# ChanukyaVardhan/Video-Moment-Localization

Hardware: AMD Instinct MI355X
Metric: proposals/sec (fwd+bwd) (higher is better)
Workload: dtype f32; 1 GPU; activitynet_t256: SMIN T=256 L=64 C=4 d=512 dl=128 Nq=20 Din=500 layers=3, batch 64/GPU, default init seed 43; step = zero_grad+fwd+restated loss+bwd+Adam (torch fused); global_batch=64, parallelism=dp1, dist_world_size=1

## Files before the change

include/smin_hip.h:

```cpp
#ifndef SMIN_HIP_H
#define SMIN_HIP_H
#include <stddef.h>
#include <stdint.h>

#ifdef __cplusplus
extern "C" {
#endif

#define SMIN_HIP_ABI_VERSION 2

int smin_abi_version(void);
int smin_set_gemm_mode(int mode);
int smin_get_gemm_mode(void);
#define SMIN_PROF_MOMENT_FWD 1
#define SMIN_PROF_MOMENT_DX 2
#define SMIN_PROF_MOMENT_DW 3
#define SMIN_PROF_ATTN_FWD 4
#define SMIN_PROF_ATTN_BWD 5
int smin_prof_enable(int on);
int smin_prof_read(int32_t* tags, float* ms, int cap);
const char* smin_target_arch(void);
size_t smin_workspace_bytes(int N, int B, int C, int D, int dl, int Nq);

int smin_proposal_map_fwd(void* stream, const float* f, const int32_t* cells, int N, int B, int T, int L, int C, int D,
// ... 155 lines not shown
                              int N, int B, int L, int C, int dl, int Nq,
                              const float* Mq, const float* uq, const float* what, const float* shat, const float* qmask,
                              uint16_t* cc_h, float* ccmean);
int smin_content_attn_fwd_probs(void* stream, const float* chat, const int32_t* cells, const int32_t* row_ptr,
                                int N, int B, int L, int C, int dl, int Nq,
                                const float* Mq, const float* uq, const float* what, const float* shat, const float* qmask,
                                void* cc, int cc_bf16, float* ccmean, float* probs);
int smin_content_attn_maps_dense(void* stream, const float* probs, const int32_t* cellmap, const int32_t* cells,
                                 int B, int L, int C, int dl, int Nq, const float* uq, const float* qmask, float* out);
#define SMIN_ATTN_MAPS_MAX_LAYERS 8
int smin_attn_maps_gather(void* stream, const float* const* probs, const float* const* bmaps, int nl, const int32_t* cellmap,
                          const int64_t* idx, int B, int L, int C, int Nq, int k, float* content, float* boundary);
size_t smin_content_attn_bwd_workspace_bytes(int N, int B, int C, int dl);
int smin_content_attn_bwd(void* stream, const float* dcc, const float* dccmean, const float* chat,
                          const int32_t* cells, const int32_t* row_ptr, int N, int B, int L, int C, int dl, int Nq,
                          const float* Mq, const float* uq, const float* what, const float* shat, const float* qmask,
                          float* dchat, float* dMq, float* duq, float* dwhat, float* dshat, void* ws, size_t ws_bytes);

int smin_linear_rows_fwd(void* stream, const float* const* xs, int nseg, const float* W, const float* bias, const float* add_rows,
                         const float* add_cells, int C, int R, int O, int K, float* y);
size_t smin_linear_rows_bwd_workspace_bytes(int R, int O, int Ktot);
int smin_linear_rows_bwd(void* stream, const float* dy, const float* const* xs, int nseg, const float* WT, int R, int O, int K,
                         float* const* dxs, float* dW, float* dbias, void* ws, size_t ws_bytes);
int smin_linear_rows_fwd_xh(void* stream, const uint16_t* const* xs, int nseg, const float* W, const float* bias, const float* add_rows,
                            const float* add_cells, int C, int R, int O, int K, float* y);
int smin_linear_rows_bwd_xh(void* stream, const float* dy, const uint16_t* const* xs, int nseg, int R, int O, int K,
                            float* dW, float* dbias, void* ws, size_t ws_bytes);
int smin_linear_rows_dx_acc(void* stream, const float* dy, int nseg, const float* WT, int R, int O, int K, float* const* dxs);
int smin_group_sum(void* stream, const float* x, int groups, int C, int W, float* out);

int smin_word_prep_fwd(void* stream, const float* fw, const float* fs, const float* qmask, const float* const* params, int nl, int B, int Nq, int D,
                       int dl, float* what, float* shat, float* kb, float* Mq, float* uq);
size_t smin_word_prep_bwd_workspace_bytes(int nl, int B, int Nq, int D, int dl);
int smin_word_prep_bwd(void* stream, const float* const* dwhat, const float* const* dshat, const float* const* dMq, const float* const* duq,
                       const float* fw, const float* fs, const float* qmask, const float* what, const float* kb, const float* const* params,
                       int nl, int B, int Nq, int D, int dl, float* dfw, float* dfs, float* const* dparams, void* ws, size_t ws_bytes);

int smin_video_encoder_fwd(void* stream, const float* x, const float* W, const float* bias, const float* pe, const float* vmask,
                           const float* fs, int B, int T, int Din, int D, float* fv, float* f);
int smin_video_encoder_gate(void* stream, const float* fv, const float* fs, int B, int T, int D, float* f);
size_t smin_video_encoder_bwd_workspace_bytes(int B, int T, int Din, int D);
int smin_video_encoder_bwd(void* stream, const float* df, const float* fv, const float* fs, const float* vmask, const float* x,
                           int B, int T, int Din, int D, float* dW, float* dbias, float* dpe, float* dfs, void* ws, size_t ws_bytes);
int smin_video_encoder_bwd_input(void* stream, const float* WT, const float* vmask, int B, int T, int Din, int D, float* dx,
                                 const void* ws, size_t ws_bytes);

int smin_sentence_feature_fwd(void* stream, const float* fw, const int32_t* len, int B, int Nq, int H, float* fs);
int smin_sentence_feature_bwd(void* stream, const float* dfs, const int32_t* len, int B, int Nq, int H, float* dfw);
int smin_lstm_pack(void* stream, const float* const* w, int In, int H, float* Wih, float* bias, float* Whh, float* W4);
int smin_lstm_pack_layers(void* stream, int nlayers, const float* const* w, const int* In, int H, float* const* Wih, float* const* bias,
                          float* const* Whh, float* const* W4);
int smin_bilstm_layer_fwd(void* stream, const float* X, const float* Wih_cat, const float* bias_cat, const float* W4,
                          const int32_t* len, int B, int Nq, int In, int H, float* G, float* Hout, float* Cs);
size_t smin_bilstm_layer_bwd_workspace_bytes(int B, int Nq, int In, int H);
int smin_bilstm_layer_bwd(void* stream, const float* dHout, const float* X, const float* Hout, const float* G, const float* Cs,
                          const float* Wih_catT, const float* Whh, const int32_t* len, int B, int Nq, int In, int H,
                          float* dX, float* dWih_cat, float* dbias_cat, float* dWhh, void* ws, size_t ws_bytes);
int smin_bilstm_layer_bwd_weights(void* stream, int which, const float* X, const float* Hout, int B, int Nq, int In, int H,
                                  float* dWih_cat, float* dbias_cat, float* dbias_cat2, float* dWhh, void* ws, size_t ws_bytes);

int smin_lstm_cluster_error(void);

int smin_build_cells(void* stream, const uint8_t* mask, int B, int L, int all_cells,
                     int32_t* cells, int32_t* row_ptr, int32_t* cellmap);
int smin_build_cells_n(void* stream, const uint8_t* mask, int B, int L, int all_cells, int n_expected,
                       int32_t* cells, int32_t* row_ptr, int32_t* cellmap, int32_t* status);
// ... 78 lines not shown
```

video-moment-localization_amd/csrc/torch_binding.cpp:

```cpp
#include <ATen/ATen.h>
#include <c10/hip/HIPGuard.h>
#include <c10/hip/HIPStream.h>
#include <hip/hip_runtime_api.h>
#include <torch/csrc/autograd/custom_function.h>
#include <torch/library.h>
#include <ATen/core/dispatch/Dispatcher.h>
#include <ATen/core/stack.h>

#include <cmath>
#include <map>
#include <mutex>
#include <tuple>
#include <vector>

#include "smin_hip.h"

namespace {

using at::Tensor;
using torch::autograd::AutogradContext;
using torch::autograd::variable_list;
using HStream = c10::hip::HIPStream;

#define SMIN_CK(call)                                                                           \
// ... 957 lines not shown
                    auto ws = scratch(smin_linear_rows_bwd_workspace_bytes(n, dl, D), dev);
                    SMIN_CK(smin_linear_rows_bwd(cur(), fp(dhp), xs, 1, nullptr, n, dl, D, nullptr, fpm(dWch), nullptr, ws.p, ws.n));
                    if (prep_kernel) base_ch[k] = dWch; else acc(dprm.layer(k, L_CH_W), dWch);
                }
            }
            {
                std::vector<Tensor> later;
                for (int64_t kk = k + 1; kk < nl; ++kk) later.push_back(dHs[kk]);
                std::vector<const float*> dh{fp(dcum)}, dr{fp(dfm)};
                Tensor later_sum;
                if (later.size() <= 3) for (auto& t : later) dh.push_back(fp(t));
                else { later_sum = sum_list(later); dh.push_back(fp(later_sum)); }
                if (k == 0) dr.push_back(fp(dcum));
                Tensor dfm_k = at::empty({N, D}, opt), dfs = at::empty_like(fs);
                auto ws = scratch((size_t)4 * B * 512 * D + 4096, dev);
                SMIN_CK(smin_gate_bwd(cur(), dh.data(), i32(dh.size()), dr.data(), i32(dr.size()), fp(ls.fm), fp(fs), ip(row_ptr), n, B, Li, D, fpm(dfm_k), fpm(dfs), ws.p, ws.n,
                                      ip(cells), fp(ls.A), fp(dbu)));
                dfs_parts.push_back(dfs);
                dfm = dfm_k;
            }
            dcum_next = dcum; dfb_next = dfb_k;
        }

        hipStreamCaptureStatus capture = hipStreamCaptureStatusNone;
        TORCH_CHECK(hipStreamIsCapturing(curs.stream(), &capture) == hipSuccess, "hipStreamIsCapturing failed");
        const bool tail_split = (flags & F_TAIL_SPLIT) && capture == hipStreamCaptureStatusNone;
        HStream tail = (flags & F_OVERLAP_PREP) ? side_stream(dev.index()) : curs;
        HStream wordst = !(flags & F_OVERLAP_PREP) ? curs : tail_split ? side_stream(dev.index(), 1) : tail;
        HStream cw = tail_split ? tail : curs;
        if (!attn0_done) attn0_done = mark(curs);
        hipEvent_t words_done;
        if (!tail_split) wait_stream(wordst, curs);
        else if (wordst != curs) await(wordst, attn0_done);
        {
            StreamScope sc(wordst);
            std::vector<const float*> gp[4], pp;
            std::vector<float*> dp;
            for (int64_t k = 0; k < nl; ++k) {
                gp[0].push_back(fp(dwhat[k])); gp[1].push_back(fp(dshat[k])); gp[2].push_back(fp(dMq[k])); gp[3].push_back(fp(duq[k]));
                for (int which : L_WORD_SIDE) {
                    pp.push_back(fp(P.layer(k, which)));
                    dprm.layer(k, which) = at::empty_like(P.layer(k, which));
                    dp.push_back(fpm(dprm.layer(k, which)));
                }
            }
            Tensor dfw = at::empty_like(fw), dfs = at::empty_like(fs);
            auto ws = scratch(smin_word_prep_bwd_workspace_bytes(i32(nl), B, Nq, D, dl), dev);
            SMIN_CK(smin_word_prep_bwd(cur(), gp[0].data(), gp[1].data(), gp[2].data(), gp[3].data(), fp(fw), fp(fs), fp(qmf), fp(st.what), fp(st.kb), pp.data(), i32(nl), B, Nq, D,
                                       dl, fpm(dfw), fpm(dfs), dp.data(), ws.p, ws.n));
            dfw_parts.push_back(dfw); dfs_parts.push_back(dfs);
            words_done = mark(wordst);
            if (sync.on) {
                std::vector<Tensor> ws_grads = loc_bufs;
                for (int64_t k = 0; k < nl; ++k)
                    for (int which : L_WORD_SIDE) ws_grads.push_back(dprm.layer(k, which));
                sync.reduce(ws_grads, wordst);
            }
        }

        Tensor df;
        hipEvent_t weights_done;
        bool tab_built = false;
        auto tab = clip_event_table(dev, Ti, Li, Ci, &tab_built);
        if (tab_built) wait_stream(cw, curs);
        {
            std::vector<const float*> ptrs;
            for (int64_t k = 0; k < nl; ++k) ptrs.push_back(fp(dchat[k]));
            if (cw != curs) await(cw, attn0_done);
            hipEvent_t dg_done;
            Tensor dg;
            {
                StreamScope sc(cw);
                dg = at::empty({(int64_t)B * T, nl * dl}, opt);
                keep.push_back(dg);
                auto ws = scratch((size_t)4 * B * T * std::max<int64_t>(D, nl * dl), dev);
                SMIN_CK(smin_clip_window_means_bwd(cur(), ptrs.data(), ip(cells), ip(row_ptr), ip(cellmap), n, B, Ti, Li, Ci, dl, i32(nl), fpm(dg), ws.p, ws.n, ip(tab.first),
                                                   tab.second.data_ptr()));
                dg_done = mark(cw);
            }
            if (!tail_split) wait_stream(wstr, curs);
            {
                StreamScope sc(tail_split ? tail : wstr);
                if (!prep_kernel) dconsts[0] = at::empty({dl}, opt);
                const float* xs[1] = {fp(f)};
// ... 455 lines not shown
```

video-moment-localization_amd/csrc/word_prep.hip:

```cpp
#include "common.h"
#include "smin_hip.h"

namespace smin {

constexpr int WP_MAXL = 8;
struct WordParams { const float* p[WP_MAXL * 8]; };
struct WordGrads { float* p[WP_MAXL * 8]; };
struct WordOuts { const float* dwhat[WP_MAXL]; const float* dshat[WP_MAXL]; const float* dMq[WP_MAXL]; const float* duq[WP_MAXL]; };

template <class F>
__device__ __forceinline__ void rows_matT(const float* in, int ldi, int nrows, const float* __restrict__ W, int O, int K, F store)
{
    const int t = threadIdx.x, G = 256 / O > 0 ? 256 / O : 1;
    const int o = t % O, g = t / O;
    if (g >= G || o >= O) return;
    float acc[16];
#pragma unroll
    for (int i = 0; i < 16; ++i) acc[i] = 0.f;
    const float* wrow = W + (size_t)o * K;
    int k = 0;
    for (; k + 32 <= K; k += 32) {
        float4 w4[8];
#pragma unroll
        for (int u = 0; u < 8; ++u) w4[u] = ldg4(wrow + k + 4 * u);
// ... 58 lines not shown
{
    extern __shared__ __attribute__((aligned(16))) float wp_smem[];
    const int b = blockIdx.x, k = blockIdx.y, t = threadIdx.x;
    const int r0 = blockIdx.z * rpp, nr = min(Nq, r0 + rpp) - r0;
    if (nr <= 0) return;
    const float *WH = P.p[8 * k], *bWH = P.p[8 * k + 1], *SH = P.p[8 * k + 2], *bSH = P.p[8 * k + 3], *AK = P.p[8 * k + 4], *bAK = P.p[8 * k + 5],
                *AQ = P.p[8 * k + 6], *bAQ = P.p[8 * k + 7];
    float* fwS = wp_smem;
    float* whS = fwS + (rpp + 1) * D;
    float* kbS = whS + rpp * dl;
    for (int idx = t * 4; idx < nr * D; idx += 1024) stg4(fwS + idx, ldg4(fw + ((size_t)b * Nq + r0) * D + idx));
    for (int idx = t * 4; idx < D; idx += 1024) stg4(fwS + rpp * D + idx, ldg4(fs + (size_t)b * D + idx));
    __syncthreads();
    const size_t ob = (((size_t)k * B + b) * Nq + r0) * dl;
    rows_matT(fwS, D, nr, WH, dl, D, [&](int w, int e, float v) {
        v = (v + bWH[e]) * qmask[(size_t)b * Nq + r0 + w];
        whS[w * dl + e] = v; what[ob + (size_t)w * dl + e] = v;
    });
    if (blockIdx.z == 0) rows_matT(fwS + rpp * D, D, 1, SH, dl, D, [&](int, int e, float v) { shat[((size_t)k * B + b) * dl + e] = v + bSH[e]; });
    __syncthreads();
    rows_matT(whS, dl, nr, AK, dl, dl, [&](int w, int e, float v) {
        v += bAK[e];
        kbS[w * dl + e] = v; kb[ob + (size_t)w * dl + e] = v;
    });
    __syncthreads();
    rows_mat(kbS, dl, nr, AQ, dl, dl, [&](int w, int d, float v) { Mq[ob + (size_t)w * dl + d] = v; });
    if (t < nr) {
        float s = 0.f;
        for (int e = 0; e < dl; ++e) s = fmaf(kbS[t * dl + e], bAQ[e], s);
        uq[((size_t)k * B + b) * Nq + r0 + t] = s;
    }
}

__host__ __device__ inline size_t wp_slab_floats(int D, int dl) { return (size_t)2 * dl * dl + (size_t)dl * D + 3 * (size_t)dl; }

__global__ __launch_bounds__(256)
void word_prep_bwd_kernel(WordOuts G, const float* __restrict__ fw, const float* __restrict__ fs, const float* __restrict__ qmask,
                          const float* __restrict__ what, const float* __restrict__ kb, WordParams P, int B, int Nq, int D, int dl, int rpp,
                          float* __restrict__ dfw_part, float* __restrict__ dfs_part, float* __restrict__ slab)
{
    extern __shared__ __attribute__((aligned(16))) float wp_smem[];
    const int b = blockIdx.x, k = blockIdx.y, t = threadIdx.x;
    const int r0 = blockIdx.z * rpp, Nw = min(Nq, r0 + rpp) - r0;
    if (Nw <= 0) return;
    const float *WH = P.p[8 * k], *SH = P.p[8 * k + 2], *AK = P.p[8 * k + 4], *AQ = P.p[8 * k + 6], *bAQ = P.p[8 * k + 7];
    const int nd = Nw * dl, ndp = rpp * dl;
    float* fwS = wp_smem;
    float* dMqS = fwS + rpp * D;
    float* kbS = dMqS + ndp;
    float* whS = kbS + ndp;
    float* dkbS = whS + ndp;
    float* dpreS = dkbS + ndp;
    float* duS = dpreS + ndp;
    float* dshS = duS + 32;
    const size_t ob = (((size_t)k * B + b) * Nq + r0) * dl, ogb = ((size_t)b * Nq + r0) * dl;
    const float* dMq = G.dMq[k]; const float* duq = G.duq[k]; const float* dwh = G.dwhat[k]; const float* dsh = G.dshat[k];
    for (int idx = t * 4; idx < Nw * D; idx += 1024) stg4(fwS + idx, ldg4(fw + ((size_t)b * Nq + r0) * D + idx));
    for (int idx = t * 4; idx < nd; idx += 1024) {
        stg4(dMqS + idx, dMq ? ldg4(dMq + ogb + idx) : f4zero());
        stg4(kbS + idx, ldg4(kb + ob + idx));
        stg4(whS + idx, ldg4(what + ob + idx));
    }
    if (t < 32) duS[t] = (duq && t < Nw) ? duq[(size_t)b * Nq + r0 + t] : 0.f;
    for (int e = t; e < dl; e += 256) dshS[e] = dsh ? dsh[(size_t)b * dl + e] : 0.f;
    __syncthreads();
    rows_matT(dMqS, dl, Nw, AQ, dl, dl, [&](int w, int e, float v) { dkbS[w * dl + e] = fmaf(duS[w], bAQ[e], v); });
    __syncthreads();
    rows_mat(dkbS, dl, Nw, AK, dl, dl, [&](int w, int c, float v) {
        if (dwh) v += dwh[ogb + w * dl + c];
        dpreS[w * dl + c] = v * qmask[(size_t)b * Nq + r0 + w];
    });
    __syncthreads();
    rows_mat(dpreS, dl, Nw, WH, dl, D, [&](int w, int d, float v) { dfw_part[(((size_t)k * B + b) * Nq + r0 + w) * D + d] = v; });
    if (blockIdx.z == 0) rows_mat(dshS, dl, 1, SH, dl, D, [&](int, int d, float v) { dfs_part[((size_t)k * B + b) * D + d] = v; });
    const int Nq_ = Nw;
    float* sl = slab + (((size_t)k * B + b) * gridDim.z + blockIdx.z) * wp_slab_floats(D, dl);
    float* sAQ = sl; float* sbAQ = sAQ + dl * dl; float* sAK = sbAQ + dl; float* sbAK = sAK + dl * dl; float* sWH = sbAK + dl; float* sbWH = sWH + (size_t)dl * D;
    for (int idx = t; idx < dl * dl; idx += 256) {
        const int e = idx / dl, c = idx % dl;
        float a = 0.f, a2 = 0.f;
        for (int w = 0; w < Nq_; ++w) { a = fmaf(kbS[w * dl + e], dMqS[w * dl + c], a); a2 = fmaf(dkbS[w * dl + e], whS[w * dl + c], a2); }
        sAQ[idx] = a; sAK[idx] = a2;
    }
    for (int e = t; e < dl; e += 256) {
        float a = 0.f, a2 = 0.f, a3 = 0.f;
        for (int w = 0; w < Nq_; ++w) { a = fmaf(kbS[w * dl + e], duS[w], a); a2 += dkbS[w * dl + e]; a3 += dpreS[w * dl + e]; }
        sbAQ[e] = a; sbAK[e] = a2; sbWH[e] = a3;
    }
    for (int idx = t * 4; idx < dl * D; idx += 1024) {
        const int e = idx / D, d = idx % D;
        float4 a = f4zero();
        for (int w = 0; w < Nq_; ++w) a = f4fma(ldg4(fwS + w * D + d), dpreS[w * dl + e], a);
        stg4(sWH + idx, a);
    }
}

__global__ __launch_bounds__(256)
void word_prep_reduce_kernel(const float* __restrict__ slab, const float* __restrict__ dfw_part, const float* __restrict__ dfs_part, WordOuts G,
                             const float* __restrict__ fs, WordGrads Q, int nl, int B, int Nq, int D, int dl, int parts, float* __restrict__ dfw,
                             float* __restrict__ dfs)
{
    const int k = blockIdx.y;
    const size_t x = (size_t)blockIdx.x * 256 + threadIdx.x;
    if (k == nl) {
        const size_t nfw = (size_t)B * Nq * D, nfs = (size_t)B * D;
        if (x < nfw) { float s = 0.f; for (int l = 0; l < nl; ++l) s += dfw_part[(size_t)l * nfw + x]; dfw[x] = s; }
        else if (x < nfw + nfs) { const size_t y = x - nfw; float s = 0.f; for (int l = 0; l < nl; ++l) s += dfs_part[(size_t)l * nfs + y]; dfs[y] = s; }
        return;
    }
    const size_t ss = wp_slab_floats(D, dl);
    float* dWH = Q.p[8 * k]; float* dbWH = Q.p[8 * k + 1]; float* dSH = Q.p[8 * k + 2]; float* dbSH = Q.p[8 * k + 3]; float* dAK = Q.p[8 * k + 4];
    float* dbAK = Q.p[8 * k + 5]; float* dAQ = Q.p[8 * k + 6]; float* dbAQ = Q.p[8 * k + 7];
    if (x < ss) {
        const float* p = slab + (size_t)k * B * parts * ss + x;
        const int P = B * parts;
        float a[8] = {0.f, 0.f, 0.f, 0.f, 0.f, 0.f, 0.f, 0.f};
        int b = 0;
        for (; b + 8 <= P; b += 8) {
#pragma unroll
            for (int u = 0; u < 8; ++u) a[u] += p[(size_t)(b + u) * ss];
        }
        for (; b < P; ++b) a[0] += p[(size_t)b * ss];
        const float s = ((a[0] + a[1]) + (a[2] + a[3])) + ((a[4] + a[5]) + (a[6] + a[7]));
        const size_t o1 = (size_t)dl * dl, o2 = o1 + dl, o3 = o2 + o1, o4 = o3 + dl, o5 = o4 + (size_t)dl * D;
        if (x < o1) dAQ[x] = s; else if (x < o2) dbAQ[x - o1] = s; else if (x < o3) dAK[x - o2] = s; else if (x < o4) dbAK[x - o3] = s;
        else if (x < o5) dWH[x - o4] = s; else dbWH[x - o5] = s;
    } else if (x < ss + (size_t)dl * D) {
        const size_t y = x - ss; const int e = (int)(y / D), d = (int)(y % D);
        const float* dsh = G.dshat[k];
        float s = 0.f;
        if (dsh) for (int b = 0; b < B; ++b) s = fmaf(dsh[(size_t)b * dl + e], fs[(size_t)b * D + d], s);
        dSH[y] = s;
    } else if (x < ss + (size_t)dl * D + dl) {
        const int e = (int)(x - ss - (size_t)dl * D);
        const float* dsh = G.dshat[k];
        float s = 0.f;
        if (dsh) for (int b = 0; b < B; ++b) s += dsh[(size_t)b * dl + e];
        dbSH[e] = s;
    }
}

}

using namespace smin;

static size_t wp_fwd_lds(int rpp, int D, int dl) { return sizeof(float) * ((size_t)(rpp + 1) * D + 2 * (size_t)rpp * dl); }
static size_t wp_bwd_lds(int rpp, int D, int dl) { return sizeof(float) * ((size_t)rpp * D + 5 * (size_t)rpp * dl + 32 + dl); }
constexpr size_t WP_MAX_LDS = 160 * 1024;
static int wp_rows_per_part(int nl, int B, int Nq, int D, int dl)
{
    int parts = cdiv(384, nl * B);
    if (parts > Nq) parts = Nq;
    if (parts < 1) parts = 1;
    while (parts < Nq && (wp_fwd_lds(cdiv(Nq, parts), D, dl) > WP_MAX_LDS || wp_bwd_lds(cdiv(Nq, parts), D, dl) > WP_MAX_LDS)) ++parts;
    return cdiv(Nq, parts);
}

extern "C" int smin_word_prep_fwd(void* stream, const float* fw, const float* fs, const float* qmask, const float* const* params, int nl, int B, int Nq, int D,
                                  int dl, float* what, float* shat, float* kb, float* Mq, float* uq)
{
    if (B == 0) return 0;
    const int rpp = wp_rows_per_part(nl, B, Nq, D, dl), parts = cdiv(Nq, rpp);
    SMIN_REQUIRE(nl >= 1 && nl <= WP_MAXL && Nq >= 1 && Nq <= 32 && D % 4 == 0 && dl % 4 == 0 && dl <= 128 && wp_fwd_lds(rpp, D, dl) <= WP_MAX_LDS);
    WordParams P;
    for (int i = 0; i < WP_MAXL * 8; ++i) P.p[i] = params[i < nl * 8 ? i : 0];
    const size_t lds = wp_fwd_lds(rpp, D, dl);
    if (lds > 64 * 1024)
        if (int e = lds_optin(reinterpret_cast<const void*>(&word_prep_fwd_kernel), lds)) return e;
    hipLaunchKernelGGL(word_prep_fwd_kernel, dim3(B, nl, parts), dim3(256), lds, (hipStream_t)stream, fw, fs, qmask, P, B, Nq, D, dl, rpp, what, shat, kb, Mq, uq);
    SMIN_LAUNCH_CHECK();
    return 0;
}

extern "C" size_t smin_word_prep_bwd_workspace_bytes(int nl, int B, int Nq, int D, int dl)
{
    const int parts = B > 0 ? cdiv(Nq, wp_rows_per_part(nl, B, Nq, D, dl)) : 1;
    return sizeof(float) * ((size_t)nl * B * parts * wp_slab_floats(D, dl) + (size_t)nl * B * Nq * D + (size_t)nl * B * D + 64);
}

extern "C" int smin_word_prep_bwd(void* stream, const float* const* dwhat, const float* const* dshat, const float* const* dMq, const float* const* duq,
                                  const float* fw, const float* fs, const float* qmask, const float* what, const float* kb, const float* const* params,
                                  int nl, int B, int Nq, int D, int dl, float* dfw, float* dfs, float* const* dparams, void* ws, size_t ws_bytes)
{
    hipStream_t st = (hipStream_t)stream;
    if (B == 0) return 0;
    const int rpp = wp_rows_per_part(nl, B, Nq, D, dl), parts = cdiv(Nq, rpp);
    SMIN_REQUIRE(nl >= 1 && nl <= WP_MAXL && Nq >= 1 && Nq <= 32 && D % 4 == 0 && dl % 4 == 0 && dl <= 128 && wp_bwd_lds(rpp, D, dl) <= WP_MAX_LDS);
    SMIN_REQUIRE(ws_bytes >= smin_word_prep_bwd_workspace_bytes(nl, B, Nq, D, dl));
    WordParams P; WordGrads Q; WordOuts G;
    for (int i = 0; i < WP_MAXL * 8; ++i) { P.p[i] = params[i < nl * 8 ? i : 0]; Q.p[i] = dparams[i < nl * 8 ? i : 0]; }
    for (int k = 0; k < WP_MAXL; ++k) {
        G.dwhat[k] = k < nl ? dwhat[k] : nullptr; G.dshat[k] = k < nl ? dshat[k] : nullptr; G.dMq[k] = k < nl ? dMq[k] : nullptr; G.duq[k] = k < nl ? duq[k] : nullptr;
    }
    float* slab = reinterpret_cast<float*>(ws);
    float* dfw_part = slab + (size_t)nl * B * parts * wp_slab_floats(D, dl);
    float* dfs_part = dfw_part + (size_t)nl * B * Nq * D;
    const size_t lds = wp_bwd_lds(rpp, D, dl);
    if (lds > 64 * 1024)
        if (int e = lds_optin(reinterpret_cast<const void*>(&word_prep_bwd_kernel), lds)) return e;
    hipLaunchKernelGGL(word_prep_bwd_kernel, dim3(B, nl, parts), dim3(256), lds, st, G, fw, fs, qmask, what, kb, P, B, Nq, D, dl, rpp, dfw_part, dfs_part, slab);
    SMIN_LAUNCH_CHECK();
    const size_t per_layer = wp_slab_floats(D, dl) + (size_t)dl * D + dl, rows = (size_t)B * Nq * D + (size_t)B * D;
    const size_t mx = per_layer > rows ? per_layer : rows;
    hipLaunchKernelGGL(word_prep_reduce_kernel, dim3((unsigned)((mx + 255) / 256), nl + 1), dim3(256), 0, st, slab, dfw_part, dfs_part, G, fs, Q, nl, B, Nq, D, dl, parts,
                       dfw, dfs);
    SMIN_LAUNCH_CHECK();
    return 0;
}
```

Measured before the change: 15.32 million proposals/s.

## Split word-prep backward into MFMA row-gradient and grouped weight-gradient kernels

Replaces the per-(batch,layer,part) word-prep backward kernel with two pieces. One MFMA kernel tiles 32 rows across all batch×query rows and accumulates dfw/dfs over layers directly, which removes the dfw/dfs partial buffers and their reduction. A grouped MFMA weight-gradient kernel then computes the parameter gradients with split-K slabs that a reduce kernel sums. The binding runs the weight-gradient part on a separate stream once row gradients are done, so it can overlap other backward work. This costs a larger workspace allocated per call and extra stream and event bookkeeping.

```diff
diff --git a/include/smin_hip.h b/include/smin_hip.h
--- a/include/smin_hip.h
+++ b/include/smin_hip.h
@@ -211,6 +211,11 @@
 int smin_word_prep_fwd(void* stream, const float* fw, const float* fs, const float* qmask, const float* const* params, int nl, int B, int Nq, int D,
                        int dl, float* what, float* shat, float* kb, float* Mq, float* uq);
 size_t smin_word_prep_bwd_workspace_bytes(int nl, int B, int Nq, int D, int dl);
+int smin_word_prep_bwd_rows(void* stream, const float* const* dwhat, const float* const* dshat, const float* const* dMq, const float* const* duq,
+                            const float* qmask, const float* const* params, int nl, int B, int Nq, int D, int dl, float* dfw,
+                            float* dfs, void* ws, size_t ws_bytes);
+int smin_word_prep_bwd_weights(void* stream, const float* const* dshat, const float* const* dMq, const float* const* duq, const float* fw, const float* fs, const float* what,
+                               const float* kb, int nl, int B, int Nq, int D, int dl, float* const* dparams, void* ws, size_t ws_bytes);
 int smin_word_prep_bwd(void* stream, const float* const* dwhat, const float* const* dshat, const float* const* dMq, const float* const* duq,
                        const float* fw, const float* fs, const float* qmask, const float* what, const float* kb, const float* const* params,
                        int nl, int B, int Nq, int D, int dl, float* dfw, float* dfs, float* const* dparams, void* ws, size_t ws_bytes);
diff --git a/video-moment-localization_amd/csrc/torch_binding.cpp b/video-moment-localization_amd/csrc/torch_binding.cpp
--- a/video-moment-localization_amd/csrc/torch_binding.cpp
+++ b/video-moment-localization_amd/csrc/torch_binding.cpp
@@ -1013,24 +1013,35 @@
         hipEvent_t words_done;
         if (!tail_split) wait_stream(wordst, curs);
         else if (wordst != curs) await(wordst, attn0_done);
+        const bool words_split = tail_split && wordst != curs && wordst != tail && wstr != curs && wstr != wordst && !sync.on;
+        HStream wwst = words_split ? wstr : wordst;
         {
-            StreamScope sc(wordst);
             std::vector<const float*> gp[4], pp;
             std::vector<float*> dp;
-            for (int64_t k = 0; k < nl; ++k) {
-                gp[0].push_back(fp(dwhat[k])); gp[1].push_back(fp(dshat[k])); gp[2].push_back(fp(dMq[k])); gp[3].push_back(fp(duq[k]));
+            Tensor wsw;
+            {
+                StreamScope sc(wordst);
+                for (int64_t k = 0; k < nl; ++k) {
+                    gp[0].push_back(fp(dwhat[k])); gp[1].push_back(fp(dshat[k])); gp[2].push_back(fp(dMq[k])); gp[3].push_back(fp(duq[k]));
+                    for (int which : L_WORD_SIDE) pp.push_back(fp(P.layer(k, which)));
+                }
+                Tensor dfw = at::empty_like(fw), dfs = at::empty_like(fs);
+                wsw = at::empty({(int64_t)smin_word_prep_bwd_workspace_bytes(i32(nl), B, Nq, D, dl) + 256}, at::TensorOptions().dtype(at::kByte).device(dev));
+                keep.push_back(wsw);
+                SMIN_CK(smin_word_prep_bwd_rows(cur(), gp[0].data(), gp[1].data(), gp[2].data(), gp[3].data(), fp(qmf), pp.data(), i32(nl), B, Nq, D, dl,
+                                                fpm(dfw), fpm(dfs), wsw.data_ptr(), (size_t)wsw.numel()));
+                dfw_parts.push_back(dfw); dfs_parts.push_back(dfs);
+                words_done = mark(wordst);
+            }
+            if (wwst != wordst) await(wwst, words_done);
+            StreamScope sc(wwst);
+            for (int64_t k = 0; k < nl; ++k)
                 for (int which : L_WORD_SIDE) {
-                    pp.push_back(fp(P.layer(k, which)));
                     dprm.layer(k, which) = at::empty_like(P.layer(k, which));
                     dp.push_back(fpm(dprm.layer(k, which)));
                 }
-            }
-            Tensor dfw = at::empty_like(fw), dfs = at::empty_like(fs);
-            auto ws = scratch(smin_word_prep_bwd_workspace_bytes(i32(nl), B, Nq, D, dl), dev);
-            SMIN_CK(smin_word_prep_bwd(cur(), gp[0].data(), gp[1].data(), gp[2].data(), gp[3].data(), fp(fw), fp(fs), fp(qmf), fp(st.what), fp(st.kb), pp.data(), i32(nl), B, Nq, D,
-                                       dl, fpm(dfw), fpm(dfs), dp.data(), ws.p, ws.n));
-            dfw_parts.push_back(dfw); dfs_parts.push_back(dfs);
-            words_done = mark(wordst);
+            SMIN_CK(smin_word_prep_bwd_weights(cur(), gp[1].data(), gp[2].data(), gp[3].data(), fp(fw), fp(fs), fp(st.what), fp(st.kb), i32(nl), B, Nq, D, dl, dp.data(),
+                                               wsw.data_ptr(), (size_t)wsw.numel()));
             if (sync.on) {
                 std::vector<Tensor> ws_grads = loc_bufs;
                 for (int64_t k = 0; k < nl; ++k)
diff --git a/video-moment-localization_amd/csrc/word_prep.hip b/video-moment-localization_amd/csrc/word_prep.hip
--- a/video-moment-localization_amd/csrc/word_prep.hip
+++ b/video-moment-localization_amd/csrc/word_prep.hip
@@ -114,112 +114,246 @@
     }
 }
 
+constexpr int WP_RT = 32;
+
+template <bool BT>
+__device__ __forceinline__ void tile_mma(f32x16& acc, const float* X, int ldx, const float* __restrict__ W, int ldw, int K, int col, int l31, int h)
+{
+    for (int k0 = 0; k0 < K; k0 += 16) {
+        float4 a[2], b[2];
+#pragma unroll
+        for (int u = 0; u < 2; ++u) {
+            const int k = k0 + 8 * u + 4 * h;
+            const bool ok = k < K;
+            const int kc = ok ? k : K - 4;
+            a[u] = ldg4(X + l31 * ldx + kc);
+            const unsigned o = BT ? (unsigned)(col * ldw + kc) : (unsigned)(kc * ldw + col), sw = (unsigned)ldw;
+            if (BT) b[u] = ldg4(W + o);
+            else b[u] = make_float4(W[o], W[o + sw], W[o + 2 * sw], W[o + 3 * sw]);
+            if (!ok) { a[u] = f4zero(); b[u] = f4zero(); }
+        }
+#pragma unroll
+        for (int u = 0; u < 2; ++u) {
+            acc = __builtin_amdgcn_mfma_f32_32x32x2f32(a[u].x, b[u].x, acc, 0, 0, 0);
+            acc = __builtin_amdgcn_mfma_f32_32x32x2f32(a[u].y, b[u].y, acc, 0, 0, 0);
+            acc = __builtin_amdgcn_mfma_f32_32x32x2f32(a[u].z, b[u].z, acc, 0, 0, 0);
+            acc = __builtin_amdgcn_mfma_f32_32x32x2f32(a[u].w, b[u].w, acc, 0, 0, 0);
+        }
+    }
+}
+
+__global__ __launch_bounds__(256, 4)
+void word_prep_bwd_kernel(WordOuts G, const float* __restrict__ qmask, WordParams P, int nl, int M, int B, int D, int dl, int word_tiles,
+                          float* __restrict__ dkb, float* __restrict__ dpre, float* __restrict__ dfw, float* __restrict__ dfs)
+{
+    extern __shared__ __attribute__((aligned(16))) float wp_smem[];
+    const int ldx = dl + 4;
+    float* Y = wp_smem;
+    float* S = Y + WP_RT * ldx;
+    float* duS = S + WP_RT * ldx;
+    float* qmS = duS + WP_RT;
+    const int t = threadIdx.x, wave = t >> 6, lane = t & 63, l31 = lane & 31, h = lane >> 5;
+    const bool words = (int)blockIdx.x < word_tiles;
+    const int r0 = (words ? blockIdx.x : blockIdx.x - word_tiles) * WP_RT;
+    const int nr = min(WP_RT, (words ? M : B) - r0);
+    const int nt = (dl + 31) / 32, widx = words ? 0 : 2;
+    const int col3 = (blockIdx.y * 4 + wave) * 32 + l31, col3c = min(col3, D - 1);
+    f32x16 acc3;
+#pragma unroll
+    for (int r = 0; r < 16; ++r) acc3[r] = 0.f;
+    if (words && t < WP_RT) qmS[t] = qmask[r0 + min(t, nr - 1)];
+    for (int l = 0; l < nl; ++l) {
+        const float* src = words ? G.dMq[l] : G.dshat[l];
+        for (int idx = t * 4; idx < WP_RT * dl; idx += 1024) {
+            const int w = idx / dl, c = idx - w * dl;
+            stg4(S + w * ldx + c, (src && w < nr) ? ldg4(src + (size_t)(r0 + w) * dl + c) : f4zero());
+        }
+        if (words && t < WP_RT) duS[t] = (G.duq[l] && t < nr) ? G.duq[l][r0 + t] : 0.f;
+        __syncthreads();
+        if (words) {
+            const float *AK = P.p[8 * l + 4], *AQ = P.p[8 * l + 6], *bAQ = P.p[8 * l + 7];
+            const float* dwh = G.dwhat[l];
+            float* dkb_t = dkb + ((size_t)l * M + r0) * dl;
+            float* dpre_t = dpre + ((size_t)l * M + r0) * dl;
+            const float* dwh_t = dwh ? dwh + (size_t)r0 * dl : nullptr;
+            for (int tile = wave; tile < nt; tile += 4) {
+                const int col = tile * 32 + l31, colc = min(col, dl - 1);
+                f32x16 acc;
+#pragma unroll
+                for (int r = 0; r < 16; ++r) acc[r] = 0.f;
+                tile_mma<true>(acc, S, ldx, AQ, dl, dl, colc, l31, h);
+                const float bq = bAQ[colc];
+#pragma unroll
+                for (int r = 0; r < 16; ++r) {
+                    const int row = (r & 3) + 8 * (r >> 2) + 4 * h;
+                    const float v = fmaf(duS[row], bq, acc[r]);
+                    if (col < dl) {
+                        Y[row * ldx + col] = v;
+                        if (blockIdx.y == 0 && row < nr) dkb_t[(unsigned)(row * dl + col)] = v;
+                    }
+                }
+            }
+            __syncthreads();
+            for (int tile = wave; tile < nt; tile += 4) {
+                const int col = tile * 32 + l31, colc = min(col, dl - 1);
+                f32x16 acc;
+#pragma unroll
+                for (int r = 0; r < 16; ++r) acc[r] = 0.f;
+                tile_mma<false>(acc, Y, ldx, AK, dl, dl, colc, l31, h);
+#pragma unroll
+                for (int r = 0; r < 16; ++r) {
+                    const int row = (r & 3) + 8 * (r >> 2) + 4 * h, rowc = min(row, nr - 1);
+                    float v = acc[r];
+                    if (dwh_t) v += dwh_t[(unsigned)(rowc * dl + colc)];
+                    v *= qmS[row];
+                    if (col < dl) {
+                        S[row * ldx + col] = v;
+                        if (blockIdx.y == 0 && row < nr) dpre_t[(unsigned)(row * dl + col)] = v;
+                    }
+                }
+            }
+            __syncthreads();
+        }
+        if (col3 - l31 < D) tile_mma<false>(acc3, S, ldx, P.p[8 * l + widx], D, dl, col3c, l31, h);
+        __syncthreads();
+    }
+    float* out = (words ? dfw : dfs) + (size_t)r0 * D;
+#pragma unroll
+    for (int r = 0; r < 16; ++r) {
+        const int row = (r & 3) + 8 * (r >> 2) + 4 * h;
+        if (row < nr && col3 < D) out[(unsigned)(row * D + col3)] = acc3[r];
+    }
+}
+
+constexpr int WP_SPLITS = 16;
+struct WgProb {
+    const float* A; const float* Bm;
+    float* out; float* bias;
+    const float* wv;
+    int M, I, J, rps, tiles_i, blk0, blk1, flags;
+};
+constexpr int WG_B_ABSENT = 1, WG_WV = 2;
+struct WgTable { WgProb p[WP_MAXL * 4]; int n; int zstride; };
+
+__global__ __launch_bounds__(256)
+void word_prep_wgrad_kernel(WgTable T)
+{
+    constexpr int BI = 128, BJ = 128, BK = 16;
+    __shared__ __attribute__((aligned(16))) float smem[BK * (BI + BJ)];
+    float* As = smem;
+    float* Bs = smem + BK * BI;
+    int q = 0;
+    while (q + 1 < T.n && (int)blockIdx.x >= T.p[q].blk1) ++q;
+    const WgProb pr = T.p[q];
+    const int I = pr.I, J = pr.J, tiles_i = pr.tiles_i, tiles_j = (J + BJ - 1) / BJ;
+    const int id = blockIdx.x - pr.blk0, tiles = tiles_i * tiles_j;
+    const int z = id / tiles, tile = id % tiles, ti = tile % tiles_i, tj = tile / tiles_i;
+    const int m_begin = min(z * pr.rps, pr.M), m_end = min(pr.M, m_begin + pr.rps);
+    const int t = threadIdx.x, lk = t >> 5, c4 = (t & 31) * 4;
+    const int ia = min(ti * BI + c4, I - 4), jb = min(tj * BJ + c4, J - 4);
+    const int wave = t >> 6, lane = t & 63, wm = wave >> 1, wn = wave & 1, l31 = lane & 31, h = lane >> 5;
+    f32x16 acc[2][2];
+#pragma unroll
+    for (int a = 0; a < 2; ++a)
+#pragma unroll
+        for (int b = 0; b < 2; ++b)
+#pragma unroll
+            for (int r = 0; r < 16; ++r) acc[a][b][r] = 0.f;
+    float4 bacc = f4zero();
+    const int nk = (m_end - m_begin + BK - 1) / BK;
+    float4 ra[2], rb[2];
+    float rw[2];
+    const bool b_on = !(pr.flags & WG_B_ABSENT), weighted = (pr.flags & WG_WV) != 0;
+    const float* Bp = b_on ? pr.Bm : pr.A;
+    auto g_load = [&](int kt) {
+#pragma unroll
+        for (int p = 0; p < 2; ++p) {
+            const int m = m_begin + kt * BK + lk + 8 * p;
+            const bool ok = m < m_end;
+            const int mc = min(m, m_end - 1);
+            const float4 a = ldg4(pr.A + (size_t)mc * I + ia), bv = ldg4(Bp + (size_t)mc * J + jb);
+            const bool okb = ok && b_on;
+            ra[p] = make_float4(ok ? a.x : 0.f, ok ? a.y : 0.f, ok ? a.z : 0.f, ok ? a.w : 0.f);
+            rb[p] = make_float4(okb ? bv.x : 0.f, okb ? bv.y : 0.f, okb ? bv.z : 0.f, okb ? bv.w : 0.f);
+            rw[p] = !weighted ? 1.f : pr.wv ? pr.wv[mc] : 0.f;
+        }
+    };
+    if (nk > 0) g_load(0);
+    for (int kt = 0; kt < nk; ++kt) {
+        __syncthreads();
+#pragma unroll
+        for (int p = 0; p < 2; ++p) {
+            bacc = f4fma(ra[p], rw[p], bacc);
+            stg4(As + (lk + 8 * p) * BI + c4, ra[p]);
+            stg4(Bs + (lk + 8 * p) * BJ + c4, rb[p]);
+        }
+        __syncthreads();
+        if (kt + 1 < nk) g_load(kt + 1);
+        const float* ab = As + wm * 64 + l31;
+        const float* bb = Bs + wn * 64 + l31;
+#pragma unroll
+        for (int s = 0; s < BK / 2; ++s) {
+            const int kk = 2 * s + h;
+            const float a0 = ab[kk * BI], a1 = ab[kk * BI + 32];
+            const float b0 = bb[kk * BJ], b1 = bb[kk * BJ + 32];
+            acc[0][0] = __builtin_amdgcn_mfma_f32_32x32x2f32(a0, b0, acc[0][0], 0, 0, 0);
+            acc[0][1] = __builtin_amdgcn_mfma_f32_32x32x2f32(a0, b1, acc[0][1], 0, 0, 0);
+            acc[1][0] = __builtin_amdgcn_mfma_f32_32x32x2f32(a1, b0, acc[1][0], 0, 0, 0);
+            acc[1][1] = __builtin_amdgcn_mfma_f32_32x32x2f32(a1, b1, acc[1][1], 0, 0, 0);
+        }
+    }
+    float* out = pr.out + (size_t)z * T.zstride;
+#pragma unroll
+    for (int mi = 0; mi < 2; ++mi)
+#pragma unroll
+        for (int ni = 0; ni < 2; ++ni)
+#pragma unroll
+            for (int r = 0; r < 16; ++r) {
+                const int i = ti * BI + wm * 64 + mi * 32 + (r & 3) + 8 * (r >> 2) + 4 * h;
+                const int j = tj * BJ + wn * 64 + ni * 32 + l31;
+                if (i < I && j < J) out[(size_t)i * J + j] = acc[mi][ni][r];
+            }
+    if (pr.bias) {
+        __syncthreads();
+        float4* red = reinterpret_cast<float4*>(smem);
+        red[lk * 32 + (t & 31)] = bacc;
+        __syncthreads();
+        if (tj == 0 && t < 32) {
+            float4 sum = red[t];
+#pragma unroll
+            for (int g = 1; g < 8; ++g) sum = f4add(sum, red[g * 32 + t]);
+            const int i0 = ti * BI + 4 * t;
+            if (ia == i0) {
+                float* o = pr.bias + (size_t)z * T.zstride + i0;
+                o[0] = sum.x; o[1] = sum.y; o[2] = sum.z; o[3] = sum.w;
+            }
+        }
+    }
+}
+
 __host__ __device__ inline size_t wp_slab_floats(int D, int dl) { return (size_t)2 * dl * dl + (size_t)dl * D + 3 * (size_t)dl; }
 
 __global__ __launch_bounds__(256)
-void word_prep_bwd_kernel(WordOuts G, const float* __restrict__ fw, const float* __restrict__ fs, const float* __restrict__ qmask,
-                          const float* __restrict__ what, const float* __restrict__ kb, WordParams P, int B, int Nq, int D, int dl, int rpp,
-                          float* __restrict__ dfw_part, float* __restrict__ dfs_part, float* __restrict__ slab)
-{
-    extern __shared__ __attribute__((aligned(16))) float wp_smem[];
-    const int b = blockIdx.x, k = blockIdx.y, t = threadIdx.x;
-    const int r0 = blockIdx.z * rpp, Nw = min(Nq, r0 + rpp) - r0;
-    if (Nw <= 0) return;
-    const float *WH = P.p[8 * k], *SH = P.p[8 * k + 2], *AK = P.p[8 * k + 4], *AQ = P.p[8 * k + 6], *bAQ = P.p[8 * k + 7];
-    const int nd = Nw * dl, ndp = rpp * dl;
-    float* fwS = wp_smem;
-    float* dMqS = fwS + rpp * D;
-    float* kbS = dMqS + ndp;
-    float* whS = kbS + ndp;
-    float* dkbS = whS + ndp;
-    float* dpreS = dkbS + ndp;
-    float* duS = dpreS + ndp;
-    float* dshS = duS + 32;
-    const size_t ob = (((size_t)k * B + b) * Nq + r0) * dl, ogb = ((size_t)b * Nq + r0) * dl;
-    const float* dMq = G.dMq[k]; const float* duq = G.duq[k]; const float* dwh = G.dwhat[k]; const float* dsh = G.dshat[k];
-    for (int idx = t * 4; idx < Nw * D; idx += 1024) stg4(fwS + idx, ldg4(fw + ((size_t)b * Nq + r0) * D + idx));
-    for (int idx = t * 4; idx < nd; idx += 1024) {
-        stg4(dMqS + idx, dMq ? ldg4(dMq + ogb + idx) : f4zero());
-        stg4(kbS + idx, ldg4(kb + ob + idx));
-        stg4(whS + idx, ldg4(what + ob + idx));
-    }
-    if (t < 32) duS[t] = (duq && t < Nw) ? duq[(size_t)b * Nq + r0 + t] : 0.f;
-    for (int e = t; e < dl; e += 256) dshS[e] = dsh ? dsh[(size_t)b * dl + e] : 0.f;
-    __syncthreads();
-    rows_matT(dMqS, dl, Nw, AQ, dl, dl, [&](int w, int e, float v) { dkbS[w * dl + e] = fmaf(duS[w], bAQ[e], v); });
-    __syncthreads();
-    rows_mat(dkbS, dl, Nw, AK, dl, dl, [&](int w, int c, float v) {
-        if (dwh) v += dwh[ogb + w * dl + c];
-        dpreS[w * dl + c] = v * qmask[(size_t)b * Nq + r0 + w];
-    });
-    __syncthreads();
-    rows_mat(dpreS, dl, Nw, WH, dl, D, [&](int w, int d, float v) { dfw_part[(((size_t)k * B + b) * Nq + r0 + w) * D + d] = v; });
-    if (blockIdx.z == 0) rows_mat(dshS, dl, 1, SH, dl, D, [&](int, int d, float v) { dfs_part[((size_t)k * B + b) * D + d] = v; });
-    const int Nq_ = Nw;
-    float* sl = slab + (((size_t)k * B + b) * gridDim.z + blockIdx.z) * wp_slab_floats(D, dl);
-    float* sAQ = sl; float* sbAQ = sAQ + dl * dl; float* sAK = sbAQ + dl; float* sbAK = sAK + dl * dl; float* sWH = sbAK + dl; float* sbWH = sWH + (size_t)dl * D;
-    for (int idx = t; idx < dl * dl; idx += 256) {
-        const int e = idx / dl, c = idx % dl;
-        float a = 0.f, a2 = 0.f;
-        for (int w = 0; w < Nq_; ++w) { a = fmaf(kbS[w * dl + e], dMqS[w * dl + c], a); a2 = fmaf(dkbS[w * dl + e], whS[w * dl + c], a2); }
-        sAQ[idx] = a; sAK[idx] = a2;
-    }
-    for (int e = t; e < dl; e += 256) {
-        float a = 0.f, a2 = 0.f, a3 = 0.f;
-        for (int w = 0; w < Nq_; ++w) { a = fmaf(kbS[w * dl + e], duS[w], a); a2 += dkbS[w * dl + e]; a3 += dpreS[w * dl + e]; }
-        sbAQ[e] = a; sbAK[e] = a2; sbWH[e] = a3;
-    }
-    for (int idx = t * 4; idx < dl * D; idx += 1024) {
-        const int e = idx / D, d = idx % D;
-        float4 a = f4zero();
-        for (int w = 0; w < Nq_; ++w) a = f4fma(ldg4(fwS + w * D + d), dpreS[w * dl + e], a);
-        stg4(sWH + idx, a);
-    }
-}
-
-__global__ __launch_bounds__(256)
-void word_prep_reduce_kernel(const float* __restrict__ slab, const float* __restrict__ dfw_part, const float* __restrict__ dfs_part, WordOuts G,
-                             const float* __restrict__ fs, WordGrads Q, int nl, int B, int Nq, int D, int dl, int parts, float* __restrict__ dfw,
-                             float* __restrict__ dfs)
+void word_prep_reduce_kernel(const float* __restrict__ slab, WordGrads Q, int splits, int D, int dl)
 {
     const int k = blockIdx.y;
     const size_t x = (size_t)blockIdx.x * 256 + threadIdx.x;
-    if (k == nl) {
-        const size_t nfw = (size_t)B * Nq * D, nfs = (size_t)B * D;
-        if (x < nfw) { float s = 0.f; for (int l = 0; l < nl; ++l) s += dfw_part[(size_t)l * nfw + x]; dfw[x] = s; }
-        else if (x < nfw + nfs) { const size_t y = x - nfw; float s = 0.f; for (int l = 0; l < nl; ++l) s += dfs_part[(size_t)l * nfs + y]; dfs[y] = s; }
-        return;
-    }
     const size_t ss = wp_slab_floats(D, dl);
-    float* dWH = Q.p[8 * k]; float* dbWH = Q.p[8 * k + 1]; float* dSH = Q.p[8 * k + 2]; float* dbSH = Q.p[8 * k + 3]; float* dAK = Q.p[8 * k + 4];
-    float* dbAK = Q.p[8 * k + 5]; float* dAQ = Q.p[8 * k + 6]; float* dbAQ = Q.p[8 * k + 7];
-    if (x < ss) {
-        const float* p = slab + (size_t)k * B * parts * ss + x;
-        const int P = B * parts;
-        float a[8] = {0.f, 0.f, 0.f, 0.f, 0.f, 0.f, 0.f, 0.f};
-        int b = 0;
-        for (; b + 8 <= P; b += 8) {
-#pragma unroll
-            for (int u = 0; u < 8; ++u) a[u] += p[(size_t)(b + u) * ss];
-        }
-        for (; b < P; ++b) a[0] += p[(size_t)b * ss];
-        const float s = ((a[0] + a[1]) + (a[2] + a[3])) + ((a[4] + a[5]) + (a[6] + a[7]));
-        const size_t o1 = (size_t)dl * dl, o2 = o1 + dl, o3 = o2 + o1, o4 = o3 + dl, o5 = o4 + (size_t)dl * D;
-        if (x < o1) dAQ[x] = s; else if (x < o2) dbAQ[x - o1] = s; else if (x < o3) dAK[x - o2] = s; else if (x < o4) dbAK[x - o3] = s;
-        else if (x < o5) dWH[x - o4] = s; else dbWH[x - o5] = s;
-    } else if (x < ss + (size_t)dl * D) {
-        const size_t y = x - ss; const int e = (int)(y / D), d = (int)(y % D);
-        const float* dsh = G.dshat[k];
-        float s = 0.f;
-        if (dsh) for (int b = 0; b < B; ++b) s = fmaf(dsh[(size_t)b * dl + e], fs[(size_t)b * D + d], s);
-        dSH[y] = s;
-    } else if (x < ss + (size_t)dl * D + dl) {
-        const int e = (int)(x - ss - (size_t)dl * D);
-        const float* dsh = G.dshat[k];
-        float s = 0.f;
-        if (dsh) for (int b = 0; b < B; ++b) s += dsh[(size_t)b * dl + e];
-        dbSH[e] = s;
-    }
+    float* dWH = Q.p[8 * k]; float* dbWH = Q.p[8 * k + 1]; float* dAK = Q.p[8 * k + 4]; float* dbAK = Q.p[8 * k + 5]; float* dAQ = Q.p[8 * k + 6];
+    float* dbAQ = Q.p[8 * k + 7];
+    if (x >= ss) return;
+    const float* p = slab + (size_t)k * splits * ss + x;
+    float a[8] = {0.f, 0.f, 0.f, 0.f, 0.f, 0.f, 0.f, 0.f};
+    int b = 0;
+    for (; b + 8 <= splits; b += 8) {
+#pragma unroll
+        for (int u = 0; u < 8; ++u) a[u] += p[(size_t)(b + u) * ss];
+    }
+    for (; b < splits; ++b) a[0] += p[(size_t)b * ss];
+    const float s = ((a[0] + a[1]) + (a[2] + a[3])) + ((a[4] + a[5]) + (a[6] + a[7]));
+    const size_t o1 = (size_t)dl * dl, o2 = 2 * o1, o3 = o2 + (size_t)dl * D, o4 = o3 + dl, o5 = o4 + dl;
+    if (x < o1) dAQ[x] = s; else if (x < o2) dAK[x - o1] = s; else if (x < o3) dWH[x - o2] = s; else if (x < o4) dbAK[x - o3] = s;
+    else if (x < o5) dbWH[x - o4] = s; else dbAQ[x - o5] = s;
 }
 
 }
@@ -227,16 +361,18 @@
 using namespace smin;
 
 static size_t wp_fwd_lds(int rpp, int D, int dl) { return sizeof(float) * ((size_t)(rpp + 1) * D + 2 * (size_t)rpp * dl); }
-static size_t wp_bwd_lds(int rpp, int D, int dl) { return sizeof(float) * ((size_t)rpp * D + 5 * (size_t)rpp * dl + 32 + dl); }
+static size_t wp_part_lds(int rpp, int D, int dl) { return sizeof(float) * ((size_t)rpp * D + 5 * (size_t)rpp * dl + 32 + dl); }
+static size_t wp_bwd_lds(int dl) { return sizeof(float) * ((size_t)2 * WP_RT * (dl + 4) + 2 * WP_RT); }
 constexpr size_t WP_MAX_LDS = 160 * 1024;
 static int wp_rows_per_part(int nl, int B, int Nq, int D, int dl)
 {
     int parts = cdiv(384, nl * B);
     if (parts > Nq) parts = Nq;
     if (parts < 1) parts = 1;
-    while (parts < Nq && (wp_fwd_lds(cdiv(Nq, parts), D, dl) > WP_MAX_LDS || wp_bwd_lds(cdiv(Nq, parts), D, dl) > WP_MAX_LDS)) ++parts;
+    while (parts < Nq && (wp_fwd_lds(cdiv(Nq, parts), D, dl) > WP_MAX_LDS || wp_part_lds(cdiv(Nq, parts), D, dl) > WP_MAX_LDS)) ++parts;
     return cdiv(Nq, parts);
 }
+static int wp_splits(int M) { const int s = cdiv(M, 32); return s > WP_SPLITS ? WP_SPLITS : s; }
 
 extern "C" int smin_word_prep_fwd(void* stream, const float* fw, const float* fs, const float* qmask, const float* const* params, int nl, int B, int Nq, int D,
                                   int dl, float* what, float* shat, float* kb, float* Mq, float* uq)
@@ -254,38 +390,95 @@
     return 0;
 }
 
+namespace {
+struct WpWs { float *dkb, *dpre, *slab; int splits; size_t floats; };
+WpWs wp_ws(void* ws, int nl, int B, int Nq, int D, int dl)
+{
+    WpWs w;
+    w.splits = B > 0 ? wp_splits(B * Nq) : 1;
+    const size_t rows = (size_t)nl * B * Nq * dl;
+    w.dkb = reinterpret_cast<float*>(ws);
+    w.dpre = w.dkb + rows;
+    w.slab = w.dpre + rows;
+    w.floats = 2 * rows + (size_t)nl * w.splits * wp_slab_floats(D, dl);
+    return w;
+}
+bool wp_dims_ok(int nl, int B, int Nq, int D, int dl)
+{
+    return nl >= 1 && nl <= WP_MAXL && Nq >= 1 && Nq <= 32 && D >= 4 && D % 4 == 0 && dl >= 4 && dl % 4 == 0 && dl <= 128 && B >= 0 &&
+           (long long)B * Nq < (1ll << 30);
+}
+}
+
 extern "C" size_t smin_word_prep_bwd_workspace_bytes(int nl, int B, int Nq, int D, int dl)
 {
-    const int parts = B > 0 ? cdiv(Nq, wp_rows_per_part(nl, B, Nq, D, dl)) : 1;
-    return sizeof(float) * ((size_t)nl * B * parts * wp_slab_floats(D, dl) + (size_t)nl * B * Nq * D + (size_t)nl * B * D + 64);
+    return sizeof(float) * wp_ws(nullptr, nl, B, Nq, D, dl).floats;
+}
+
+extern "C" int smin_word_prep_bwd_rows(void* stream, const float* const* dwhat, const float* const* dshat, const float* const* dMq, const float* const* duq,
+                                       const float* qmask, const float* const* params, int nl, int B, int Nq, int D, int dl, float* dfw,
+                                       float* dfs, void* ws, size_t ws_bytes)
+{
+    if (B == 0) return 0;
+    SMIN_REQUIRE(wp_dims_ok(nl, B, Nq, D, dl));
+    SMIN_REQUIRE(ws_bytes >= smin_word_prep_bwd_workspace_bytes(nl, B, Nq, D, dl));
+    const WpWs w = wp_ws(ws, nl, B, Nq, D, dl);
+    const size_t lds = wp_bwd_lds(dl);
+    SMIN_REQUIRE(lds <= WP_MAX_LDS);
+    WordParams P; WordOuts G;
+    for (int i = 0; i < WP_MAXL * 8; ++i) P.p[i] = params[i < nl * 8 ? i : 0];
+    for (int k = 0; k < WP_MAXL; ++k) {
+        G.dwhat[k] = k < nl ? dwhat[k] : nullptr; G.dshat[k] = k < nl ? dshat[k] : nullptr; G.dMq[k] = k < nl ? dMq[k] : nullptr; G.duq[k] = k < nl ? duq[k] : nullptr;
+    }
+    if (lds > 64 * 1024)
+        if (int e = lds_optin(reinterpret_cast<const void*>(&word_prep_bwd_kernel), lds)) return e;
+    const int M = B * Nq, word_tiles = cdiv(M, WP_RT), col_groups = cdiv(D, 128);
+    hipLaunchKernelGGL(word_prep_bwd_kernel, dim3(word_tiles + cdiv(B, WP_RT), col_groups), dim3(256), lds, (hipStream_t)stream, G, qmask, P, nl, M, B, D, dl, word_tiles,
+                       w.dkb, w.dpre, dfw, dfs);
+    SMIN_LAUNCH_CHECK();
+    return 0;
+}
+
+extern "C" int smin_word_prep_bwd_weights(void* stream, const float* const* dshat, const float* const* dMq, const float* const* duq, const float* fw, const float* fs, const float* what,
+                                          const float* kb, int nl, int B, int Nq, int D, int dl, float* const* dparams, void* ws, size_t ws_bytes)
+{
+    if (B == 0) return 0;
+    SMIN_REQUIRE(wp_dims_ok(nl, B, Nq, D, dl));
+    SMIN_REQUIRE(ws_bytes >= smin_word_prep_bwd_workspace_bytes(nl, B, Nq, D, dl));
+    const WpWs w = wp_ws(ws, nl, B, Nq, D, dl);
+    const int M = B * Nq, rps = cdiv(M, w.splits);
+    const size_t ss = wp_slab_floats(D, dl), o1 = (size_t)dl * dl, o2 = 2 * o1, o3 = o2 + (size_t)dl * D, o4 = o3 + dl, o5 = o4 + dl;
+    WgTable T;
+    WordGrads Q;
+    for (int i = 0; i < WP_MAXL * 8; ++i) Q.p[i] = dparams[i < nl * 8 ? i : 0];
+    int blk = 0, n = 0;
+    auto add = [&](const float* A, const float* Bm, float* out, float* bias, const float* wv, int flags, int rows, int I, int J, int splits, int rows_per_split) {
+        WgProb& p = T.p[n++];
+        p.A = A; p.Bm = Bm; p.out = out; p.bias = bias; p.wv = wv;
+        p.M = A ? rows : 0; p.I = I; p.J = J; p.rps = rows_per_split; p.tiles_i = cdiv(I, 128);
+        p.blk0 = blk; blk += p.tiles_i * cdiv(J, 128) * splits; p.blk1 = blk; p.flags = flags | (Bm ? 0 : WG_B_ABSENT);
+    };
+    for (int k = 0; k < nl; ++k) {
+        float* sl = w.slab + (size_t)k * w.splits * ss;
+        const size_t rows = (size_t)k * M * dl;
+        add(kb + rows, dMq[k], sl, sl + o5, duq[k], WG_WV, M, dl, dl, w.splits, rps);
+        add(w.dkb + rows, what + rows, sl + o1, sl + o3, nullptr, 0, M, dl, dl, w.splits, rps);
+        add(w.dpre + rows, fw, sl + o2, sl + o4, nullptr, 0, M, dl, D, w.splits, rps);
+        add(dshat[k], fs, dparams[8 * k + 2], dparams[8 * k + 3], nullptr, 0, B, dl, D, 1, B);
+    }
+    for (int i = n; i < WP_MAXL * 4; ++i) T.p[i] = T.p[0];
+    T.n = n; T.zstride = (int)ss;
+    hipLaunchKernelGGL(word_prep_wgrad_kernel, dim3(blk), dim3(256), 0, (hipStream_t)stream, T);
+    SMIN_LAUNCH_CHECK();
+    hipLaunchKernelGGL(word_prep_reduce_kernel, dim3((unsigned)((ss + 255) / 256), nl), dim3(256), 0, (hipStream_t)stream, w.slab, Q, w.splits, D, dl);
+    SMIN_LAUNCH_CHECK();
+    return 0;
 }
 
 extern "C" int smin_word_prep_bwd(void* stream, const float* const* dwhat, const float* const* dshat, const float* const* dMq, const float* const* duq,
                                   const float* fw, const float* fs, const float* qmask, const float* what, const float* kb, const float* const* params,
                                   int nl, int B, int Nq, int D, int dl, float* dfw, float* dfs, float* const* dparams, void* ws, size_t ws_bytes)
 {
-    hipStream_t st = (hipStream_t)stream;
-    if (B == 0) return 0;
-    const int rpp = wp_rows_per_part(nl, B, Nq, D, dl), parts = cdiv(Nq, rpp);
-    SMIN_REQUIRE(nl >= 1 && nl <= WP_MAXL && Nq >= 1 && Nq <= 32 && D % 4 == 0 && dl % 4 == 0 && dl <= 128 && wp_bwd_lds(rpp, D, dl) <= WP_MAX_LDS);
-    SMIN_REQUIRE(ws_bytes >= smin_word_prep_bwd_workspace_bytes(nl, B, Nq, D, dl));
-    WordParams P; WordGrads Q; WordOuts G;
-    for (int i = 0; i < WP_MAXL * 8; ++i) { P.p[i] = params[i < nl * 8 ? i : 0]; Q.p[i] = dparams[i < nl * 8 ? i : 0]; }
-    for (int k = 0; k < WP_MAXL; ++k) {
-        G.dwhat[k] = k < nl ? dwhat[k] : nullptr; G.dshat[k] = k < nl ? dshat[k] : nullptr; G.dMq[k] = k < nl ? dMq[k] : nullptr; G.duq[k] = k < nl ? duq[k] : nullptr;
-    }
-    float* slab = reinterpret_cast<float*>(ws);
-    float* dfw_part = slab + (size_t)nl * B * parts * wp_slab_floats(D, dl);
-    float* dfs_part = dfw_part + (size_t)nl * B * Nq * D;
-    const size_t lds = wp_bwd_lds(rpp, D, dl);
-    if (lds > 64 * 1024)
-        if (int e = lds_optin(reinterpret_cast<const void*>(&word_prep_bwd_kernel), lds)) return e;
-    hipLaunchKernelGGL(word_prep_bwd_kernel, dim3(B, nl, parts), dim3(256), lds, st, G, fw, fs, qmask, what, kb, P, B, Nq, D, dl, rpp, dfw_part, dfs_part, slab);
-    SMIN_LAUNCH_CHECK();
-    const size_t per_layer = wp_slab_floats(D, dl) + (size_t)dl * D + dl, rows = (size_t)B * Nq * D + (size_t)B * D;
-    const size_t mx = per_layer > rows ? per_layer : rows;
-    hipLaunchKernelGGL(word_prep_reduce_kernel, dim3((unsigned)((mx + 255) / 256), nl + 1), dim3(256), 0, st, slab, dfw_part, dfs_part, G, fs, Q, nl, B, Nq, D, dl, parts,
-                       dfw, dfs);
-    SMIN_LAUNCH_CHECK();
-    return 0;
-}
+    if (int e = smin_word_prep_bwd_rows(stream, dwhat, dshat, dMq, duq, qmask, params, nl, B, Nq, D, dl, dfw, dfs, ws, ws_bytes)) return e;
+    return smin_word_prep_bwd_weights(stream, dshat, dMq, duq, fw, fs, what, kb, nl, B, Nq, D, dl, dparams, ws, ws_bytes);
+}
```

Measured after the change: 15.43 million proposals/s (median of 6 runs). About the same (+0.8%).
